# gmum/3d-point-clouds-autocomplete

Measured on AMD Instinct MI355X. Metric: train-step point-clouds/sec at B=64, N=2048 (Chamfer+EMD), higher is better.
Workload: dtype f32 storage / accumulation / results; matrix products formed from f16 x2 (bf16 x3) pieces of the fp32 operands — NOT IEEE-fp32 products: the all-fp32-kernel step is `value_strict_fp32`

## Files before the change

### 3d-point-clouds-autocomplete_amd/csrc/hp_model.h

```cpp
#pragma once

#define HP_MAX_HEADS 8
#define HP_MAX_TN_LAYERS 8

typedef struct HpEncoderWeights {
    const float* conv_w[5];
    const float* conv_b[5];
    const float* fc_w;
    const float* fc_b;
    const float* mu_w;
    const float* mu_b;
    const float* std_w;
    const float* std_b;
} HpEncoderWeights;

typedef struct HpEncoderGrads {
    float* conv_w[5];
    float* conv_b[5];
    float* fc_w;
    float* fc_b;
    float* mu_w;
    float* mu_b;
    float* std_w;
    float* std_b;
} HpEncoderGrads;

typedef struct HpEncoderIO {
    const float* x;
    const HpEncoderWeights* w;
    const float* eps;
    int* argidx;
    float *g, *f, *mu, *lv, *z, *explv, *ws;
    int is_vae;
    int out_ld;
} HpEncoderIO;

typedef struct HpEncoderBwdIO {
    const float* x;
    const HpEncoderWeights* w;
    const float* eps;
    const int* argidx;
    const float *g, *f, *lv;
    const float *grad_out, *grad_mu, *grad_explv;
    const HpEncoderGrads* gr;
    float* ws;
    const float* fwd_ws;
    int is_vae;
    int grad_out_ld;
} HpEncoderBwdIO;

enum { HP_ENC_CONV_PFORMAT = 0, HP_ENC_CONV_SPLIT_F32 = 1, HP_ENC_CONV_GEMM_F32 = 2 };
typedef struct HpEncoderPlan {
    int conv_format;
    int pool_fused;
    int tile_rows;
    int fwd_tails_skinny;
    int bwd_fused;
    int bwd_splits;
    int bwd_tails_skinny[2];
} HpEncoderPlan;

typedef struct HpHyperWeights {
    const float* trunk_w[5];
    const float* trunk_b[5];
    int n_heads;
    int head_out[HP_MAX_HEADS];
    const float* head_w[HP_MAX_HEADS];
    const float* head_b[HP_MAX_HEADS];
} HpHyperWeights;

typedef struct HpHyperGrads {
    float* trunk_w[5];
    float* trunk_b[5];
    float* head_w[HP_MAX_HEADS];
    float* head_b[HP_MAX_HEADS];
} HpHyperGrads;

enum { HP_HEADS_FWD_STREAM = 0, HP_HEADS_FWD_GEMM = 1, HP_HEADS_FWD_PER_HEAD = 2 };
enum { HP_HEADS_DW_DIRECT = 0, HP_HEADS_DW_GEMM = 1, HP_HEADS_DW_PER_HEAD = 2, HP_HEADS_DW_SKIPPED = 3 };
typedef struct HpHeadsPlan {
    int fwd_route;
    int dw_route;
    int dw_rows_route;
} HpHeadsPlan;

#ifdef __cplusplus
bool hp_heads_dw_fast_ok(int cols, const float* t5, const float* out);
bool hp_heads_fwd_enabled();
int hp_heads_fwd_set(int on);
long hp_heads_fwd_ws_floats();
bool hp_heads_fwd_ok(int B, int N, int K, const float* t5, const float* W, const float* ws);
int hp_heads_fwd(int B, int N, const float* t5, const float* W, const float* bias, float* theta, int theta_ld, float* ws,
                 hipStream_t stream);
int hp_heads_dw_launch(int Kc, int rows, int r0, const float* dtheta, int theta_ld, const float* t5, int cols, float* dW,
                       float* db, hipStream_t stream);
#endif
```

### 3d-point-clouds-autocomplete_amd/csrc/model.hip

```cpp
#include "hp_common.h"
#include "hp_gemm.h"
#include "hp_conv_split.h"
#include "hp_model.h"
#include "hp_skinny.h"
#include "hp_enc_bwd.h"
#include <algorithm>
#include <cstdlib>

extern "C" int hp_gemm_f32(const HpGemmDesc* d, hipStream_t stream);
extern "C" int hp_gemm_tile_rows(const HpGemmDesc* d);
extern "C" int hp_colsum_f32(int batch, int M, int N, const float* X, long sXz, int ldx, const float* mask, long sMaskz,
                             int ldmask, float* out, long sOz, float* ws, hipStream_t stream);

namespace {

constexpr int kEnc[6] = {3, 64, 128, 256, 512, 512};
constexpr int kTrunk[5] = {64, 128, 512, 1024, 2048};
constexpr long kSplitWs = 4L << 20;

#define TRY(x)            \
    do {                  \
        int _rc = (x);    \
        if (_rc) return _rc; \
    } while (0)
// ... 977 lines not shown
                                        enc_tail_backward_program(B, out_size, 1, &t[z], pr) == 0 && hp_skinny_check(&pr) == 0;
        }
    }
    if (plan->bwd_fused) {
        HpSkProgram pr;
        const int ok = ask && enc_tail_backward_program(B, out_size, n, t, pr) == 0 && hp_skinny_check(&pr) == 0;
        for (int z = 0; z < n; ++z) plan->bwd_tails_skinny[z] = ok;
    }
    return 0;
}

namespace {
template <typename P>
bool heads_contiguous(P const* hw, P const* hb, const int* out, int n) {
    for (int h = 0; h + 1 < n; ++h)
        if (hw[h + 1] != hw[h] + (long)out[h] * 2048 || hb[h + 1] != hb[h] + out[h]) return false;
    return n > 0;
}

int trunk_forward_skinny(int B, int in_size, const float* latent, const HpHyperWeights* w, float* t, float* slabs,
                         hipStream_t stream) {
    if (B > 64 || in_size % 32) return -2;
    HpSkProgram pr{};
    HpSkSrc src{};
    src.p = latent; src.S = 1; src.ld = in_size;
    float* tl = t;
    float* sl = slabs;
    int kin = in_size;
    for (int l = 0; l < 5; ++l) {
        const int N = kTrunk[l];
        const int S = sk_ranges(kin, N / 32, 4);
        HpSkOp& op = pr.op[pr.nops++];
        op.type = HP_SK_F; op.phase = l;
        op.a = src;
        op.w = w->trunk_w[l]; op.w_ld = kin;
        op.M = B; op.N = N; op.K = kin; op.CL = kin / S;
        op.out_ld = N;
        HpSkSrc next{};
        next.ld = N;
        if (S == 1) {
            op.out = tl; op.out_bias = w->trunk_b[l]; op.out_relu = l < 4;
            next.p = tl; next.S = 1;
        } else {
            op.out = sl; op.out_slab = 64L * N;
            next.p = sl; next.slab = 64L * N; next.S = S; next.bias = w->trunk_b[l]; next.relu = l < 4;
            next.mat = tl; next.ldmat = N;
            sl += (long)S * 64 * N;
            if (sl - slabs > kSplitWs) return -2;
        }
        src = next;
        kin = N;
        tl += (long)B * N;
    }
    if (src.S > 1) {
        HpSkOp& op = pr.op[pr.nops++];
        op.type = HP_SK_FIN; op.phase = 5;
        op.out = src.mat; op.out_ld = src.ldmat;
        src.mat = nullptr;
        op.a = src;
        op.M = B; op.N = 2048; op.K = 1;
    }
    return hp_skinny_run(&pr, stream);
}

int trunk_backward_skinny(int B, int in_size, const float* latent, const HpHyperWeights* w, const float* const* act,
                          float* const* dt, const HpHyperGrads* gr, float* grad_latent, float* slabs, hipStream_t stream) {
    if (B > 64 || in_size % 32) return -2;
    HpSkProgram pr{};
    HpSkSrc src{};
    src.p = dt[4]; src.S = 1; src.ld = kTrunk[4];
    float* sl = slabs;
    int phase = 0;
    auto dw_op = [&](int l) {
        HpSkOp& op = pr.op[pr.nops++];
        op.type = HP_SK_W; op.phase = phase;
        op.a.p = dt[l]; op.a.S = 1; op.a.ld = kTrunk[l];
        op.w = l ? act[l - 1] : latent; op.w_ld = l ? kTrunk[l - 1] : in_size;
        op.out = gr->trunk_w[l]; op.out_ld = op.w_ld; op.rsum = gr->trunk_b[l];
        op.M = B; op.N = kTrunk[l]; op.K = op.w_ld;
    };
    for (int l = 4; l >= 0; --l, ++phase) {
        const int N = kTrunk[l], K = l ? kTrunk[l - 1] : in_size;
        if (l == 0 && !grad_latent) {
            HpSkOp& op = pr.op[pr.nops++];
            op.type = HP_SK_FIN; op.phase = phase;
            op.out = src.mat; op.out_ld = src.ldmat;
            src.mat = nullptr;
            op.a = src;
            op.M = B; op.N = N; op.K = 1;
        } else {
            const int S = sk_ranges(N, K / 32, 4);
            HpSkOp& op = pr.op[pr.nops++];
            op.type = HP_SK_X; op.phase = phase;
            op.a = src;
            op.w = w->trunk_w[l]; op.w_ld = K;
            op.M = B; op.N = N; op.K = K; op.CL = N / S;
            op.out_ld = K;
            HpSkSrc next{};
            next.ld = K;
            if (l == 0) {
                if (S == 1) {
                    op.out = grad_latent;
                } else {
                    op.out = sl; op.out_slab = 64L * K;
                    next.p = sl; next.slab = 64L * K; next.S = S;
                    sl += (long)S * 64 * K;
                }
            } else {
                op.out = sl; op.out_slab = 64L * K;
                next.p = sl; next.slab = 64L * K; next.S = S;
                next.mask = act[l - 1]; next.ldm = K; next.mat = dt[l - 1]; next.ldmat = K;
                sl += (long)S * 64 * K;
            }
            if (sl - slabs > kSplitWs) return -2;
            src = next;
        }
        if (l == 4) dw_op(4);
        else if (l <= 2) dw_op(l + 1);
    }
    if (grad_latent && src.p && src.S > 1) {
        HpSkOp& op = pr.op[pr.nops++];
        op.type = HP_SK_FIN; op.phase = phase;
        op.a = src;
        op.out = grad_latent; op.out_ld = in_size;
        op.M = B; op.N = in_size; op.K = 1;
    }
    dw_op(0);
    return hp_skinny_run(&pr, stream);
}

template <typename T>
inline T* hyper_splitws(T* t, int B) { return t + ((long)B * (64 + 128 + 512 + 1024 + 2048) + 3) / 4 * 4; }
inline int heads_total(const HpHyperWeights* w) {
    int total = 0;
    for (int hd = 0; hd < w->n_heads; ++hd) total += w->head_out[hd];
    return total;
}
int heads_fwd_route(int B, const HpHyperWeights* w, const float* t) {
    if (!heads_contiguous(w->head_w, w->head_b, w->head_out, w->n_heads)) return HP_HEADS_FWD_PER_HEAD;
    const float* t5 = t + (long)B * (64 + 128 + 512 + 1024);
    return hp_heads_fwd_enabled() && hp_heads_fwd_ws_floats() <= kSplitWs &&
                   hp_heads_fwd_ok(B, heads_total(w), 2048, t5, w->head_w[0], hyper_splitws(t, B))
               ? HP_HEADS_FWD_STREAM : HP_HEADS_FWD_GEMM;
}
int heads_dw_route(const HpHyperWeights* w, const HpHyperGrads* gr, const float* t5) {
    const bool skip_dw = gr->head_w[0] == nullptr;
    bool gb_contig = true;
    for (int h = 0; h + 1 < w->n_heads; ++h) gb_contig = gb_contig && gr->head_b[h + 1] == gr->head_b[h] + w->head_out[h];
    const bool w_contig = heads_contiguous(w->head_w, w->head_b, w->head_out, w->n_heads);
    if (skip_dw) return gb_contig && w_contig ? HP_HEADS_DW_SKIPPED : -1;
    if (!w_contig || !heads_contiguous(gr->head_w, gr->head_b, w->head_out, w->n_heads)) return HP_HEADS_DW_PER_HEAD;
    return hp_heads_dw_fast_ok(2048, t5, gr->head_w[0]) ? HP_HEADS_DW_DIRECT : HP_HEADS_DW_GEMM;
}
int heads_dw_rows_route(const float* t5_all, const float* dW_rows) {
    return hp_heads_dw_fast_ok(2048, t5_all, dW_rows) ? HP_HEADS_DW_DIRECT : HP_HEADS_DW_GEMM;
}
}

HP_API long hp_hypernet_saved_floats(int B) { return (long)B * (64 + 128 + 512 + 1024 + 2048) + kSplitWs + 64; }
HP_API long hp_hypernet_backward_workspace_floats(int B) { return (long)B * (64 + 128 + 512 + 1024 + 2048) + kSplitWs + 64; }

HP_API int hp_hypernet_set_heads_stream(int on) { return hp_heads_fwd_set(on); }

HP_API int hp_hypernet_forward(int B, int in_size, const float* latent, const HpHyperWeights* w, float* t, float* theta,
                               int theta_ld, hipStream_t stream) {
    HP_CHECK_ARG(B > 0 && in_size > 0 && latent && w && t && theta && w->n_heads > 0 && w->n_heads <= HP_MAX_HEADS);
    Op op{stream, hyper_splitws(t, B)};
    const float* in = latent;
    int kin = in_size;
    float* tl = t;
    int sk = hp_skinny_enabled() ? trunk_forward_skinny(B, in_size, latent, w, t, op.splitws, stream) : -2;
    if (sk != -2) {
        TRY(sk);
        in = t + (long)B * (64 + 128 + 512 + 1024);
    } else {
        for (int l = 0; l < 5; ++l) {
            TRY(op.lin_fwd(in, 0, kin, w->trunk_w[l], 0, w->trunk_b[l], 0, tl, 0, kTrunk[l], B, kTrunk[l], kin, 1, l < 4));
            in = tl;
            kin = kTrunk[l];
            tl += (long)B * kTrunk[l];
        }
    }
    const int total = heads_total(w);
    HP_CHECK_ARG(total <= theta_ld);
    switch (heads_fwd_route(B, w, t)) {
    case HP_HEADS_FWD_STREAM:
        TRY(hp_heads_fwd(B, total, in, w->head_w[0], w->head_b[0], theta, theta_ld, op.splitws, stream));
        break;
    case HP_HEADS_FWD_GEMM:
        TRY(op.lin_fwd(in, 0, 2048, w->head_w[0], 0, w->head_b[0], 0, theta, 0, theta_ld, B, total, 2048, 1, false));
        break;
    default: {
        int off = 0;
        for (int hd = 0; hd < w->n_heads; ++hd) {
            TRY(op.lin_fwd(in, 0, 2048, w->head_w[hd], 0, w->head_b[hd], 0, theta + off, 0, theta_ld, B, w->head_out[hd], 2048,
                           1, false));
            off += w->head_out[hd];
        }
    }
    }
    HP_RETURN_LAST_ERROR();
}

namespace {
int hypernet_backward_impl(int B, int in_size, const float* latent, const HpHyperWeights* w, const float* t, const float* grad_theta,
                           int theta_ld, const HpHyperGrads* gr, float* grad_latent, float* ws, hipStream_t stream, hipStream_t after);
}
HP_API int hp_hypernet_backward(int B, int in_size, const float* latent, const HpHyperWeights* w, const float* t,
                                const float* grad_theta, int theta_ld, const HpHyperGrads* gr, float* grad_latent, float* ws,
                                hipStream_t stream) {
    return hypernet_backward_impl(B, in_size, latent, w, t, grad_theta, theta_ld, gr, grad_latent, ws, stream, nullptr);
}
HP_API int hp_hypernet_backward_ordered(int B, int in_size, const float* latent, const HpHyperWeights* w, const float* t,
                                        const float* grad_theta, int theta_ld, const HpHyperGrads* gr, float* grad_latent, float* ws,
                                        hipStream_t stream, hipStream_t after) {
    return hypernet_backward_impl(B, in_size, latent, w, t, grad_theta, theta_ld, gr, grad_latent, ws, stream, after);
}
namespace {
int hypernet_backward_impl(int B, int in_size, const float* latent, const HpHyperWeights* w, const float* t, const float* grad_theta,
                           int theta_ld, const HpHyperGrads* gr, float* grad_latent, float* ws, hipStream_t stream, hipStream_t after) {
    HP_CHECK_ARG(B > 0 && in_size > 0 && latent && w && t && grad_theta && gr && ws);
    const float* act[5];
    {
        const float* tl = t;
        for (int l = 0; l < 5; ++l) {
            act[l] = tl;
            tl += (long)B * kTrunk[l];
        }
    }
    float* p = ws;
    float* dt[5];
    for (int l = 0; l < 5; ++l) {
        dt[l] = p;
        p += (long)B * kTrunk[l];
    }
    Op op{stream, p};
    int off = 0;
    const int total = heads_total(w);
    const int route = heads_dw_route(w, gr, act[4]);
    HP_CHECK_ARG(route >= 0);
    const bool fused = route != HP_HEADS_DW_PER_HEAD;
    if (fused) {
        if (route == HP_HEADS_DW_DIRECT) {
            TRY(hp_heads_dw_launch(B, total, 0, grad_theta, theta_ld, act[4], 2048, gr->head_w[0], gr->head_b[0], stream));
        } else if (route == HP_HEADS_DW_GEMM)
            TRY(op.lin_dw(grad_theta, 0, theta_ld, act[4], 0, 2048, gr->head_w[0], 0, B, total, 2048, 1, gr->head_b[0]));
        else if (gr->head_b[0])
            TRY(op.colsum(grad_theta, 0, theta_ld, B, total, 1, gr->head_b[0], 0));
        TRY(op.lin_dx(grad_theta, 0, theta_ld, w->head_w[0], 0, dt[4], 0, 2048, B, total, 2048, 1, nullptr, 0, 0, nullptr, 2048));
    }
    for (int hd = 0; hd < w->n_heads && !fused; ++hd) {
        const int nh = w->head_out[hd];
        TRY(op.lin_dw(grad_theta + off, 0, theta_ld, act[4], 0, 2048, gr->head_w[hd], 0, B, nh, 2048, 1, gr->head_b[hd]));
        TRY(op.lin_dx(grad_theta + off, 0, theta_ld, w->head_w[hd], 0, dt[4], 0, 2048, B, nh, 2048, 1, nullptr, 0, 0,
                      hd ? dt[4] : nullptr, 2048));
        off += nh;
    }
    if (after && after != stream) TRY(hp_order_streams(stream, after));
    {
        const int sk = hp_skinny_enabled() ? trunk_backward_skinny(B, in_size, latent, w, act, dt, gr, grad_latent, p, stream) : -2;
        if (sk != -2) return sk ? sk : (int)hipGetLastError();
    }
    for (int l = 4; l >= 0; --l) {
        const float* below = l ? act[l - 1] : latent;
        const int kin = l ? kTrunk[l - 1] : in_size;
        TRY(op.lin_dw(dt[l], 0, kTrunk[l], below, 0, kin, gr->trunk_w[l], 0, B, kTrunk[l], kin, 1, gr->trunk_b[l]));
        if (l > 0)
            TRY(op.lin_dx(dt[l], 0, kTrunk[l], w->trunk_w[l], 0, dt[l - 1], 0, kin, B, kTrunk[l], kin, 1, act[l - 1], 0, kin,
                          nullptr, 0));
        else if (grad_latent)
            TRY(op.lin_dx(dt[0], 0, kTrunk[0], w->trunk_w[0], 0, grad_latent, 0, kin, B, kTrunk[0], kin, 1, nullptr, 0, 0,
                          nullptr, 0));
    }
    HP_RETURN_LAST_ERROR();
}
}

HP_API long hp_hypernet_t5_offset(int B) { return (long)B * (64 + 128 + 512 + 1024); }
HP_API long hp_hypernet_heads_dw_workspace_floats(void) { return kSplitWs + 64; }
HP_API int hp_hypernet_heads_dw_rows(int Kc, int rows, int r0, const float* dtheta_all, int theta_ld, const float* t5_all,
                                     float* dW_rows, float* ws, hipStream_t stream) {
    HP_CHECK_ARG(Kc > 0 && rows >= 0 && r0 >= 0 && r0 + rows <= theta_ld && dtheta_all && t5_all && ws);
    if (rows == 0) return 0;
    HP_CHECK_ARG(dW_rows);
    if (heads_dw_rows_route(t5_all, dW_rows) == HP_HEADS_DW_DIRECT)
        return hp_heads_dw_launch(Kc, rows, r0, dtheta_all, theta_ld, t5_all, 2048, dW_rows, nullptr, stream);
    Op op{stream, ws};
    TRY(op.lin_dw(dtheta_all + r0, 0, theta_ld, t5_all, 0, 2048, dW_rows, 0, Kc, rows, 2048, 1));
    HP_RETURN_LAST_ERROR();
}

HP_API int hp_hypernet_heads_plan(int B, const HpHyperWeights* w, const HpHyperGrads* gr, const float* t, const float* dW_rows,
                                  HpHeadsPlan* plan) {
    HP_CHECK_ARG(B > 0 && w && t && plan && w->n_heads > 0 && w->n_heads <= HP_MAX_HEADS);
    const float* t5 = t + hp_hypernet_t5_offset(B);
    plan->fwd_route = heads_fwd_route(B, w, t);
    plan->dw_route = gr ? heads_dw_route(w, gr, t5) : -1;
    plan->dw_rows_route = dW_rows ? heads_dw_rows_route(t5, dW_rows) : -1;
    return gr && plan->dw_route < 0 ? -1 : 0;
}

namespace {
struct TnLayout {
    int nl;
    int cin[HP_MAX_TN_LAYERS], cout[HP_MAX_TN_LAYERS];
    long woff[HP_MAX_TN_LAYERS], boff[HP_MAX_TN_LAYERS];
    long total, act_per_point;
};
bool tn_layout(int n_hidden, const int* channels, TnLayout* L) {
    if (n_hidden < 1 || n_hidden + 1 > HP_MAX_TN_LAYERS) return false;
    L->nl = n_hidden + 1;
    long off = 0;
    L->act_per_point = 0;
    for (int l = 0; l < L->nl; ++l) {
        L->cin[l] = l ? channels[l - 1] : 3;
        L->cout[l] = l < n_hidden ? channels[l] : 3;
        L->woff[l] = off;
        off += (long)L->cin[l] * L->cout[l];
        L->boff[l] = off;
        off += L->cout[l];
        if (l < n_hidden) L->act_per_point += channels[l];
    }
    L->total = off;
    return true;
}
}

HP_API long hp_target_theta_size(int n_hidden, const int* channels) {
    TnLayout L;
    return tn_layout(n_hidden, channels, &L) ? L.total : -1;
}
HP_API long hp_target_saved_floats(int B, int N, int n_hidden, const int* channels) {
    TnLayout L;
    return tn_layout(n_hidden, channels, &L) ? (long)B * N * L.act_per_point : -1;
}
HP_API long hp_target_backward_workspace_floats(int B, int N, int n_hidden, const int* channels) {
    TnLayout L;
    return tn_layout(n_hidden, channels, &L) ? (long)B * N * L.act_per_point + kSplitWs + 64 : -1;
}

HP_API int hp_target_forward(int B, int N, int n_hidden, const int* channels, const float* theta, int theta_ld,
                             const float* pts, float* acts, float* y, hipStream_t stream) {
    TnLayout L;
    HP_CHECK_ARG(B > 0 && N > 0 && theta && pts && acts && y && tn_layout(n_hidden, channels, &L) && L.total <= theta_ld);
    Op op{stream, nullptr};
    const float* in = pts;
    float* a = acts;
    for (int l = 0; l < L.nl; ++l) {
        const bool last = (l == L.nl - 1);
        float* out = last ? y : a;
        TRY(op.lin_fwd(in, (long)N * L.cin[l], L.cin[l], theta + L.woff[l], theta_ld, theta + L.boff[l], theta_ld, out,
                       (long)N * L.cout[l], L.cout[l], N, L.cout[l], L.cin[l], B, !last));
        in = out;
        if (!last) a += (long)B * N * L.cout[l];
    }
    HP_RETURN_LAST_ERROR();
}

HP_API int hp_target_backward(int B, int N, int n_hidden, const int* channels, const float* theta, int theta_ld,
                              const float* pts, const float* acts, const float* grad_y, float* grad_theta, float* ws,
                              hipStream_t stream) {
    TnLayout L;
    HP_CHECK_ARG(B > 0 && N > 0 && theta && pts && acts && grad_y && grad_theta && ws && tn_layout(n_hidden, channels, &L) &&
                 L.total <= theta_ld);
    const float* act[HP_MAX_TN_LAYERS];
    float* dl[HP_MAX_TN_LAYERS];
    {
        const float* a = acts;
        float* p = ws;
        for (int l = 0; l < n_hidden; ++l) {
            act[l] = a;
            dl[l] = p;
            a += (long)B * N * L.cout[l];
            p += (long)B * N * L.cout[l];
        }
        ws = p;
    }
    Op op{stream, ws};
    const float* d = grad_y;
    for (int l = L.nl - 1; l >= 0; --l) {
        const float* below = l ? act[l - 1] : pts;
        const int cin = L.cin[l], cout = L.cout[l];
        TRY(op.lin_dw(d, (long)N * cout, cout, below, (long)N * cin, cin, grad_theta + L.woff[l], theta_ld, N, cout, cin, B,
                      grad_theta + L.boff[l], theta_ld));
        if (l > 0) {
            TRY(op.lin_dx(d, (long)N * cout, cout, theta + L.woff[l], theta_ld, dl[l - 1], (long)N * cin, cin, N, cout, cin, B,
                          act[l - 1], (long)N * cin, cin, nullptr, 0));
            d = dl[l - 1];
        }
    }
    HP_RETURN_LAST_ERROR();
}
```

### include/hyperpocket_hip.h

```cpp
#ifndef HYPERPOCKET_HIP_H
#define HYPERPOCKET_HIP_H

#ifdef __cplusplus
extern "C" {
#endif

typedef struct ihipStream_t* hpStream_t;


int hp_nndistance(int b, int n, const float* xyz, int m, const float* xyz2, float* result, int* result_i,
                  float* result2, int* result2_i, hpStream_t stream);

int hp_nn_set_queries_per_lane(int r);
int hp_nn_queries_per_lane(int b, int n, int m);

int hp_nndistancegrad(int b, int n, const float* xyz1, int m, const float* xyz2, const float* grad_dist1,
                      const int* idx1, const float* grad_dist2, const int* idx2, float* grad_xyz1, float* grad_xyz2,
                      hpStream_t stream);

int hp_approxmatch(int b, int n, int m, const float* xyz1, const float* xyz2, float* match, float* temp,
                   hpStream_t stream);
long hp_approxmatch_workspace_floats(int b, int n, int m);
int hp_approxmatch_ws(int b, int n, int m, const float* xyz1, const float* xyz2, float* match, float* temp, float* ws,
                      hpStream_t stream);
// ... 37 lines not shown

int hp_emd_pairs(int na, int n, const float* A, int nb, int m, const float* B, int pairs, const int* pair_ab,
                 float* temp, float* ws, float* partials, float* cost, hpStream_t stream);

#define HP_OCCUPANCY_MAX_R 64
int hp_occupancy_grid(int S, int n, const float* clouds, int R, const float* axis, const unsigned int* columns,
                      int cells, int* counters, int* clouds_hit, int* nonfinite, hpStream_t stream);
int hp_occupancy_cells_host(long count, const float* points, int R, const float* axis, const unsigned int* columns,
                            int* cell_out);

#define HP_GEMM_BIAS 1
#define HP_GEMM_RELU 2
#define HP_GEMM_MASK 4
#define HP_GEMM_ADD 8
#define HP_GEMM_ROWSUM 32
#define HP_GEMM_COLMAX 16

typedef struct HpGemmDesc {
    const float* A;
    const float* B;
    float* C;
    const float* bias;
    const float* mask;
    const float* add;
    float* ws;
    long sAz, sBz, sCz, sBiasz, sMaskz, sAddz;
    long sAi, sAk, sBk, sBj;
    int ldc, ldmask, ldadd;
    int M, N, K, batch;
    int ksplit;
    int flags;
    float* cmax;
    int* cidx;
    int group_rows;
    float* rsum;
    long sRsumz;
    const int* dyn_count;
    int dyn_kind;
} HpGemmDesc;

long hp_gemm_workspace_floats(const HpGemmDesc* d);
int hp_gemm_tile_rows(const HpGemmDesc* d);
int hp_gemm_plan(const HpGemmDesc* d, int* tile, int* mode);
int hp_gemm_f32(const HpGemmDesc* d , hpStream_t stream);
long hp_colsum_workspace_floats(int batch, int M, int N);
int hp_colsum_f32(int batch, int M, int N, const float* X, long sXz, int ldx, const float* mask, long sMaskz,
                  int ldmask, float* out, long sOz, float* ws , hpStream_t stream);

#define HP_MAX_HEADS 8
#define HP_MAX_TN_LAYERS 8

typedef struct HpEncoderWeights {
    const float* conv_w[5];
    const float* conv_b[5];
    const float* fc_w;
    const float* fc_b;
    const float* mu_w;
    const float* mu_b;
    const float* std_w;
    const float* std_b;
} HpEncoderWeights;

typedef struct HpEncoderGrads {
    float* conv_w[5];
    float* conv_b[5];
    float* fc_w;
    float* fc_b;
    float* mu_w;
    float* mu_b;
    float* std_w;
    float* std_b;
} HpEncoderGrads;

typedef struct HpHyperWeights {
    const float* trunk_w[5];
    const float* trunk_b[5];
    int n_heads;
    int head_out[HP_MAX_HEADS];
    const float* head_w[HP_MAX_HEADS];
    const float* head_b[HP_MAX_HEADS];
} HpHyperWeights;

typedef struct HpHyperGrads {
    float* trunk_w[5];
    float* trunk_b[5];
    float* head_w[HP_MAX_HEADS];
    float* head_b[HP_MAX_HEADS];
} HpHyperGrads;

long hp_encoder_forward_workspace_floats(int B, int Np);
int hp_encoder_forward(int B, int Np, const float* x, const HpEncoderWeights* w, int out_size, int is_vae,
                       const float* eps, int* argidx, float* g, float* f, float* mu, float* lv, float* z, float* explv,
                       float* ws, hpStream_t stream);
typedef struct HpEncoderIO {
    const float* x;
    const HpEncoderWeights* w;
    const float* eps;
    int* argidx;
    float *g, *f, *mu, *lv, *z, *explv, *ws;
    int is_vae;
    int out_ld;
} HpEncoderIO;
int hp_encoder_forward_pair(int B, int Np, int out_size, const HpEncoderIO* io , hpStream_t stream);
int hp_encoder_workspace_to_f32(int B, int Np, float* ws, hpStream_t stream);
int hp_conv_presplit_set(int on);
long hp_gemm_pp_workspace_floats(long M, int N, int K);
int hp_gemm_pp_prepare(long M, int N, int K, int xcb, const float* X, const float* W, float* ws, hpStream_t stream);
int hp_gemm_pp_run(long M, int N, int K, int xcb, const float* bias, int relu, int mode, int group_rows, float* ws, hpStream_t stream);
int hp_gemm_pp_unpack(long M, int N, int K, const float* ws, float* C, hpStream_t stream);
int hp_gemm_pp_partials(long M, int N, int K, const float* ws, float* cmax, int* cidx, hpStream_t stream);
long hp_encoder_backward_workspace_floats(int B, int out_size);
int hp_encoder_backward(int B, int Np, const float* x, const HpEncoderWeights* w, int out_size, int is_vae,
                        const float* eps, const int* argidx, const float* g, const float* f, const float* lv,
                        const float* grad_out, const float* grad_mu, const float* grad_explv, const HpEncoderGrads* grads,
                        float* ws, const float* fwd_ws, int dedup, hpStream_t stream);
int hp_encoder_backward_ld(int B, int Np, const float* x, const HpEncoderWeights* w, int out_size, int is_vae,
                           const float* eps, const int* argidx, const float* g, const float* f, const float* lv,
                           const float* grad_out, int grad_out_ld, const float* grad_mu, const float* grad_explv,
                           const HpEncoderGrads* grads, float* ws, const float* fwd_ws, int dedup, hpStream_t stream);
typedef struct HpEncoderBwdIO {
    const float* x;
    const HpEncoderWeights* w;
    const float* eps;
    const int* argidx;
    const float *g, *f, *lv;
    const float *grad_out, *grad_mu, *grad_explv;
    const HpEncoderGrads* gr;
    float* ws;
    const float* fwd_ws;
    int is_vae;
    int grad_out_ld;
} HpEncoderBwdIO;
int hp_encoder_backward_pair(int B, int Np, int out_size, const HpEncoderBwdIO* io , int dedup, hpStream_t stream);
enum { HP_ENC_CONV_PFORMAT = 0, HP_ENC_CONV_SPLIT_F32 = 1, HP_ENC_CONV_GEMM_F32 = 2 };
typedef struct HpEncoderPlan {
    int conv_format;
    int pool_fused;
    int tile_rows;
    int fwd_tails_skinny;
    int bwd_fused;
    int bwd_splits;
    int bwd_tails_skinny[2];
} HpEncoderPlan;
int hp_encoder_plan(int B, int Np, int out_size, int n, const int* is_vae, const int* ld, int aligned, int dedup,
                    HpEncoderPlan* plan);
int hp_encoder_backward_set_fused(int on);
int hp_encoder_backward_set_chain_f16(int on);
int hp_conv_split_set(int on);
long hp_gemm_f16x2_workspace_floats(long M, int N, int K);
int hp_gemm_f16x2_prepare(long M, int N, int K, const float* X, const float* W, float* ws, hpStream_t stream);
int hp_gemm_f16x2_run(long M, int N, int K, const float* X, const float* bias, float* C, int relu, const float* ws, hpStream_t stream);

int hp_hypernet_set_heads_stream(int on);
long hp_hypernet_saved_floats(int B);
int hp_hypernet_forward(int B, int in_size, const float* latent, const HpHyperWeights* w, float* t, float* theta,
                        int theta_ld, hpStream_t stream);
long hp_hypernet_backward_workspace_floats(int B);
int hp_hypernet_backward(int B, int in_size, const float* latent, const HpHyperWeights* w, const float* t,
                         const float* grad_theta, int theta_ld, const HpHyperGrads* grads, float* grad_latent ,
                         float* ws, hpStream_t stream);
int hp_hypernet_backward_ordered(int B, int in_size, const float* latent, const HpHyperWeights* w, const float* t,
                                 const float* grad_theta, int theta_ld, const HpHyperGrads* grads, float* grad_latent ,
                                 float* ws, hpStream_t stream, hpStream_t after);
long hp_hypernet_t5_offset(int B);
long hp_hypernet_heads_dw_workspace_floats(void);
int hp_hypernet_heads_dw_rows(int Kc, int rows, int r0, const float* dtheta_all, int theta_ld, const float* t5_all,
                              float* dW_rows, float* ws, hpStream_t stream);
enum { HP_HEADS_FWD_STREAM = 0, HP_HEADS_FWD_GEMM = 1, HP_HEADS_FWD_PER_HEAD = 2 };
enum { HP_HEADS_DW_DIRECT = 0, HP_HEADS_DW_GEMM = 1, HP_HEADS_DW_PER_HEAD = 2, HP_HEADS_DW_SKIPPED = 3 };
typedef struct HpHeadsPlan {
    int fwd_route;
    int dw_route;
    int dw_rows_route;
} HpHeadsPlan;
int hp_hypernet_heads_plan(int B, const HpHyperWeights* w, const HpHyperGrads* grads , const float* t,
                           const float* dW_rows , HpHeadsPlan* plan);

int hp_hypernet_heads_dw_adam(int Kc, int rows, int r0, const float* dtheta_all, int theta_ld, const float* t5_all,
                              float* W_rows, float* m_rows, float* v_rows, float lr, float beta1, float beta2, float eps,
                              int step, hpStream_t stream);
int hp_hypernet_heads_dw_adam_bg(int Kc, int rows, int r0, const float* dtheta_all, int theta_ld, const float* t5_all,
                                 float* W_rows, float* m_rows, float* v_rows, float lr, float beta1, float beta2, float eps,
                                 int step, int cus, hpStream_t stream);

int hp_skinny_set_enabled(int on);
long hp_skinny_programs_run(void);

long hp_target_theta_size(int n_hidden, const int* channels);
long hp_target_saved_floats(int B, int N, int n_hidden, const int* channels);
int hp_target_forward(int B, int N, int n_hidden, const int* channels, const float* theta, int theta_ld, const float* pts,
                      float* acts, float* y, hpStream_t stream);
long hp_target_backward_workspace_floats(int B, int N, int n_hidden, const int* channels);
int hp_target_backward(int B, int N, int n_hidden, const int* channels, const float* theta, int theta_ld, const float* pts,
                       const float* acts, const float* grad_y, float* grad_theta, float* ws, hpStream_t stream);

int hp_target_fused_supported(int n_hidden, const int* channels);
long hp_target_fused_workspace_floats(int B, int N);
int hp_target_fused_set_f16(int on);
int hp_target_fused_forward(int B, int N, const float* theta, int theta_ld, const float* pts, float* y, hpStream_t stream);
int hp_target_fused_backward(int B, int N, const float* theta, int theta_ld, const float* pts, const float* grad_y,
                             float* grad_theta, float* ws, hpStream_t stream);

int hp_sample_points(long total, float coef, unsigned long long seed, unsigned long long offset, float* out,
                     hpStream_t stream);
int hp_slice_clouds(int B, int N, int target, const float* pts, unsigned long long seed, int max_rounds, float* part_a,
                    float* part_b, float* plane, int* status, hpStream_t stream);
int hp_slice_clouds_planes(int B, int N, int target, const float* pts, const double* planes, int R, float* part_a,
                           float* part_b, int* plane_idx, int* status, hpStream_t stream);
long hp_make_batch_workspace_bytes(int B, int N);
int hp_make_batch(int M, int N, int target, const float* clouds, int B, const int* ids, const long long* streams,
                  const int* degrees, const float* rot, unsigned long long seed, int max_candidates, int groups,
                  float* existing, float* missing, float* gt, float* plane, int* index, int* failed, void* ws,
                  hpStream_t stream);
#define HP_SCAN_MAX_POINTS (1 << 22)
int hp_scan_boxes(int S, const float* points, const long long* offsets, float* center , float* scale ,
                  hpStream_t stream);
int hp_prepare_scans(int B, const float* points, const long long* offsets, int S, const int* ids, const long long* streams,
                     unsigned long long seed, int target, int replace, const float* center, const float* scale, float* out,
                     int* index, int* failed, hpStream_t stream);
int hp_restore_scans(int K, int N, const float* completions, const float* s_scale, const float* center, const float* scale,
                     float* out, hpStream_t stream);
#define HP_FPS_MAX_POINTS 8192
int hp_farthest_points(int B, int P, const float* clouds, const int* counts, const int* start, int k, int* index,
                       float* radius2, int* failed, hpStream_t stream);
int hp_farthest_points_plan(int P, int* threads, int* points_per_lane);
#define HP_KNN_MAX_POINTS 65536
int hp_knn_points(int S, const float* points, const long long* offsets, const float* queries, const long long* query_offsets,
                  int k, int exclude_self, int* index , float* dist2 , hpStream_t stream);
int hp_knn_points_plan(int k, int* instance_k, int* threads, int* tile);
int hp_scan_outliers(int S, const float* points, const long long* offsets, int k, float ratio, unsigned char* keep ,
                     float* mean_dist , int* kept , hpStream_t stream);
#define HP_CLUSTER_MAX_POINTS 32768
int hp_scan_clusters(int S, const float* points, const long long* offsets, float radius, int max_points,
                     int* label , int* size , int* clusters , int* largest ,
                     hpStream_t stream);
int hp_scan_clusters_plan(int max_points, int* threads, int* tile, int* lds_bytes);
#define HP_PLANE_MAX_TRIALS 4096
long hp_scan_plane_workspace_bytes(int S, int trials);
int hp_scan_plane_plan(int trials, int* threads, int* rows_per_lane, int* trial_tile);
int hp_scan_plane(int S, const float* points, const long long* offsets, const long long* streams ,
                  unsigned long long seed, int trials, float threshold, int min_inliers, float min_share,
                  int* trial , int* inliers , int* found , int* sample ,
                  float* sample_plane , unsigned char* inlier , long long* moments ,
                  int* shift , void* ws, hpStream_t stream);
int hp_scan_plane_side(int S, const float* points, const long long* offsets, const float* planes , float threshold,
                       float* dist , unsigned char* keep , int* kept , hpStream_t stream);
#define HP_VOXEL_GRID_HALF (1 << 20)
long hp_scan_voxels_workspace_bytes(long long T, int slots_per_row);
int hp_scan_voxels_plan(int* threads, int* rows_per_lane);
int hp_scan_voxels(int S, long long T, const float* points, const long long* offsets, const float* voxel ,
                   const float* origin , int keep_mode, int slots_per_row, int* label ,
                   int* size , unsigned char* keep , int* kept , int* beyond , void* ws,
                   hpStream_t stream);
#define HP_ALIGN_MAX_POINTS 65536
#define HP_ALIGN_MAX_HYPOTHESES 64
long hp_scan_align_workspace_bytes(int S, int H);
int hp_scan_align_plan(int H, int* threads, int* rows_per_lane, int* hypothesis_group, int* tile);
int hp_scan_align_step(int S, int H, long long T, const float* points, const long long* offsets, long long U,
                       const float* tpoints, const long long* toffsets, const float* transforms , float max_dist,
                       const float* anchor , const int* shift , long long* moments ,
                       int* index , float* dist2 , hpStream_t stream);
long hp_scan_align_plane_workspace_bytes(int S, int H);
int hp_scan_align_plane_plan(int H, int* threads, int* rows_per_lane, int* hypothesis_group, int* tile);
int hp_scan_align_plane_step(int S, int H, long long T, const float* points, const long long* offsets, long long U,
                             const float* tpoints, const long long* toffsets, const float* tnormals ,
                             const float* transforms , float max_dist, const float* anchor ,
                             const int* shift , long long* moments , int* index ,
                             float* dist2 , hpStream_t stream);
int hp_scan_normals_plan(int k, int* instance_k, int* threads, int* sweeps);
int hp_scan_normals(int S, const float* points, const long long* offsets, int k, const int* index ,
                    const float* viewpoints , float* normal , float* curvature ,
                    int* count , hpStream_t stream);
#define HP_AXIS_SPLIT_MAX_POINTS 8192
int hp_axis_split(int B, int n, const float* clouds , int axis, int k,
                  float* lower , float* upper , int* order ,
                  hpStream_t stream);
#define HP_MESH_MAX_FACES 32768
int hp_mesh_sample(int K, int V, const float* verts, int F, const int* faces, int n, unsigned long long seed,
                   const long long* streams , float* points , int* face ,
                   double* area , int* failed , void* ws, hpStream_t stream);
long hp_mesh_sample_workspace_bytes(int K, int F, int n);
int hp_mesh_sample_plan(int K, int F, int n, int* threads, int* slices, int* in_lds);
int hp_mesh_sample_set_slices(int s);
int hp_mesh_sample_set_lds_faces(int faces);
int hp_mesh_normals(int K, int V, const float* verts, int F, const int* faces, const int* vf_offsets, const int* vf_faces,
                    float* face_normal , float* vertex_normal , hpStream_t stream);
int hp_kld_forward(long n, int batch, const float* explv, const float* mu, float* out, hpStream_t stream);
int hp_kld_backward(long n, int batch, const float* explv, const float* mu, const float* grad_out, float* grad_explv,
                    float* grad_mu, hpStream_t stream);
int hp_step_losses(int b, const float* cd, const float* kld, const float* cost, float c_cd, float c_emd, float* out ,
                   hpStream_t stream);

int hp_adam_step(long n, float* p, const float* g, float* m, float* v, float lr, float beta1, float beta2, float eps,
                 int step, float grad_scale, hpStream_t stream);

#define HP_TSNE_MAX_POINTS 16384
int hp_pairwise_sqdist(int n, int d, const float* X, long ldx, float* D , hpStream_t stream);
int hp_pairwise_sqdist_plan(int n, int d, int* tile, int* kchunk);
long hp_tsne_affinities_workspace_floats(int n);
int hp_tsne_affinities(int n, const float* D, float perplexity, float* P , float* beta ,
                       int* steps , float* ws, hpStream_t stream);
int hp_tsne_gradient(int n, const float* P, float exaggeration, const float* Y , float* rowacc ,
                     float* kl , hpStream_t stream);
int hp_tsne_update(int n, const float* rowacc, float* Y, float* update, float* gains, float momentum, float lr,
                   float min_gain, float* grad , hpStream_t stream);
int hp_tsne_descend(int n, const float* P, float* Y, float* update, float* gains, float* rowacc, int it0, int iters,
// ... 26 lines not shown
```

Measured before the change: 28590.

## Add streaming split-K MFMA kernel for hypernetwork heads input-gradient

```diff
diff --git a/3d-point-clouds-autocomplete_amd/csrc/heads_dx.hip b/3d-point-clouds-autocomplete_amd/csrc/heads_dx.hip
--- /dev/null
+++ b/3d-point-clouds-autocomplete_amd/csrc/heads_dx.hip
@@ -0,0 +1,188 @@
+#include "hp_common.h"
+#include "hp_model.h"
+#include <type_traits>
+
+namespace {
+
+typedef float f32x16 __attribute__((ext_vector_type(16)));
+
+constexpr int kCols = 2048, kTiles = kCols / 32;
+constexpr int kWaves = 4, kThreads = kWaves * 64;
+constexpr int kChunk = 32;
+constexpr int kRing = 3;
+constexpr int kWStage = kChunk * 128;
+constexpr int kDStage = 64 * 32 * 4;
+constexpr int kStage = kWStage + kDStage;
+constexpr int kWaveLds = kRing * kStage;
+constexpr int kLds = kWaves * kWaveLds;
+constexpr int kMaxSplits = 16;
+constexpr long kSlab = 64L * kCols;
+
+__device__ __forceinline__ void glds16(const void* sbase, unsigned voff, unsigned lds_dst) {
+    unsigned keep;
+    asm volatile("s_mov_b32 %0, m0\n\ts_mov_b32 m0, %3\n\ts_nop 0\n\tglobal_load_lds_dwordx4 %1, %2\n\ts_mov_b32 m0, %0"
+                 : "=&s"(keep)
+                 : "v"(voff), "s"(sbase), "s"(lds_dst)
+                 : "memory");
+}
+
+template <int NT>
+__global__ __launch_bounds__(kThreads, 1) void heads_dx_kernel(int B, int N, int L, int splits, const float* __restrict__ dth,
+                                                                int theta_ld, const float* __restrict__ W, float* __restrict__ slabs) {
+    constexpr int kD = 4 * NT, kDma = 4 + kD;
+    __shared__ __attribute__((aligned(1024))) unsigned char lds[kLds];
+    const int tid = threadIdx.x, lane = tid & 63, w = __builtin_amdgcn_readfirstlane(tid >> 6), i = lane & 31, h = lane >> 5;
+    const int ct = blockIdx.x % kTiles, split = (blockIdx.x / kTiles) * kWaves + w;
+    if (split >= splits) return;
+    const int r_lo = min(split * L, N), r_hi = min(r_lo + L, N);
+    const int nch = (r_hi - r_lo + kChunk - 1) / kChunk;
+    auto uniform_ptr = [](const void* q) {
+        const unsigned long long p = reinterpret_cast<unsigned long long>(q);
+        const unsigned lo = __builtin_amdgcn_readfirstlane((unsigned)p), hi = __builtin_amdgcn_readfirstlane((unsigned)(p >> 32));
+        return reinterpret_cast<const void*>(((unsigned long long)hi << 32) | lo);
+    };
+    const void* wbase = uniform_ptr(W);
+    const unsigned long long dptr = reinterpret_cast<unsigned long long>(dth);
+    const void* dbase = uniform_ptr(reinterpret_cast<const void*>(dptr & ~15ull));
+    const unsigned boff = __builtin_amdgcn_readfirstlane((unsigned)(dptr & 15) >> 2);
+    const unsigned jmax = (boff + (unsigned)(B - 1) * (unsigned)theta_ld + (unsigned)(N - 1)) >> 2;
+    const unsigned wave_lds = __builtin_amdgcn_readfirstlane((unsigned)(size_t)lds + (unsigned)(w * kWaveLds));
+    const int wrow = lane >> 3;
+    const unsigned wcol = (unsigned)(ct * 128 + (lane & 7) * 16);
+    unsigned ec[kD];
+#pragma unroll
+    for (int p = 0; p < kD; ++p) {
+        const int c = 8 * p + (lane >> 3), piece = ((lane & 7) - (c >> 1)) & 7;
+        ec[p] = boff + (unsigned)min(c, B - 1) * (unsigned)theta_ld + 4u * (unsigned)piece;
+    }
+    auto issue_w = [&](int n0, unsigned st, int j) {
+        const int row = min(n0 + 8 * j + wrow, N - 1);
+        glds16(wbase, (unsigned)row * (unsigned)(kCols * 4) + wcol, st + j * 1024);
+    };
+    auto issue_d = [&](int n0, unsigned st, int p) {
+        const unsigned piece = min((ec[p] + (unsigned)n0) >> 2, jmax);
+        glds16(dbase, piece << 4, st + kWStage + p * 1024);
+    };
+    const int rb = h * 512 + i * 4;
+    int ra[NT], ph[NT], rot[NT];
+#pragma unroll
+    for (int t = 0; t < NT; ++t) {
+        const int c = 32 * t + i;
+        ra[t] = kWStage + c * 128;
+        ph[t] = (int)((boff + (unsigned)c * (unsigned)theta_ld) & 3) + 4 * h;
+        rot[t] = ph[t] + 4 * ((c >> 1) & 7);
+    }
+    f32x16 acc[NT] = {};
+    if (nch > 0) {
+        int slot_w = 0;
+#pragma unroll 1
+        for (int c = 0; c < 2; ++c) {
+            const int nw = r_lo + min(c, nch - 1) * kChunk, nd = r_lo + c * kChunk;
+            const unsigned st = wave_lds + (unsigned)(slot_w * kStage);
+#pragma unroll
+            for (int j = 0; j < 4; ++j) issue_w(nw, st, j);
+#pragma unroll
+            for (int p = 0; p < kD; ++p) issue_d(nd, st, p);
+            slot_w = slot_w == kRing - 1 ? 0 : slot_w + 1;
+        }
+        int slot_r = 0;
+#pragma unroll 1
+        for (int c = 0; c < nch; ++c) {
+            asm volatile("s_waitcnt vmcnt(%0)" ::"n"(kDma) : "memory");
+            const int n0 = r_lo + c * kChunk;
+            const int nw2 = r_lo + min(c + 2, nch - 1) * kChunk, nd2 = r_lo + min(c + 2, nch) * kChunk;
+            const unsigned st2 = wave_lds + (unsigned)(slot_w * kStage);
+            const unsigned char* st = lds + w * kWaveLds + slot_r * kStage;
+            const unsigned char* stn = lds + w * kWaveLds + (slot_r == kRing - 1 ? 0 : slot_r + 1) * kStage;
+            const int lim = r_hi - n0 - 4 * h;
+            float av[2][4][NT], bv[2][4];
+            auto read_group = [&](int g, float (&a)[4][NT], float (&b)[4]) {
+#pragma unroll
+                for (int s = 0; s < 4; ++s) {
+                    const int r0 = 8 * g + s;
+                    b[s] = *reinterpret_cast<const float*>(st + rb + r0 * 128);
+#pragma unroll
+                    for (int t = 0; t < NT; ++t) {
+                        const unsigned char* base = (g == 3 && ph[t] + r0 >= 32) ? stn : st;
+                        a[s][t] = *reinterpret_cast<const float*>(base + ra[t] + ((rot[t] + r0) & 31) * 4);
+                    }
+                }
+            };
+            auto contract = [&](auto ragged) {
+                read_group(0, av[0], bv[0]);
+#pragma unroll
+                for (int g = 0; g < 4; ++g) {
+                    if (g + 1 < 4) {
+                        if (g + 1 == 3) asm volatile("s_waitcnt vmcnt(8)" ::: "memory");
+                        read_group(g + 1, av[(g + 1) & 1], bv[(g + 1) & 1]);
+                    }
+                    __builtin_amdgcn_sched_barrier(0);
+#pragma unroll
+                    for (int s = 0; s < 4; ++s) {
+                        const int q = 4 * g + s;
+#pragma unroll
+                        for (int t = 0; t < NT; ++t) {
+                            const bool zero = decltype(ragged)::value && 8 * g + s >= lim;
+                            const float a = zero ? 0.f : av[g & 1][s][t], b = zero ? 0.f : bv[g & 1][s];
+                            acc[t] = __builtin_amdgcn_mfma_f32_32x32x2f32(a, b, acc[t], 0, 0, 0);
+                            __builtin_amdgcn_sched_barrier(0);
+                            if (t == 0 && q < kDma) {
+                                if (q < 4) issue_w(nw2, st2, q);
+                                else issue_d(nd2, st2, q - 4);
+                                __builtin_amdgcn_sched_barrier(0);
+                            }
+                        }
+                    }
+                }
+            };
+            if (n0 + kChunk > r_hi) contract(std::true_type{});
+            else contract(std::false_type{});
+            slot_w = slot_w == kRing - 1 ? 0 : slot_w + 1;
+            slot_r = slot_r == kRing - 1 ? 0 : slot_r + 1;
+        }
+    }
+    float* out = slabs + (long)split * kSlab + ct * 32 + i;
+#pragma unroll
+    for (int t = 0; t < NT; ++t)
+#pragma unroll
+        for (int e = 0; e < 16; ++e) {
+            const int row = t * 32 + (e & 3) + 8 * (e >> 2) + 4 * h;
+            if (row < B) out[(long)row * kCols] = acc[t][e];
+        }
+    asm volatile("s_waitcnt vmcnt(0)" ::: "memory");
+}
+
+__global__ __launch_bounds__(256) void heads_dx_finish_kernel(int B, int S, const float* __restrict__ slabs, float* __restrict__ out) {
+    const int idx = blockIdx.x * 256 + threadIdx.x;
+    if (idx >= B * (kCols / 4)) return;
+    const float4* p = reinterpret_cast<const float4*>(slabs) + idx;
+    float4 v = S <= 8 ? p[0] : make_float4(0.f, 0.f, 0.f, 0.f);
+    for (int s = S <= 8 ? 1 : 0; s < S; ++s) {
+        const float4 t = p[(long)s * (kSlab / 4)];
+        v = make_float4(v.x + t.x, v.y + t.y, v.z + t.z, v.w + t.w);
+    }
+    reinterpret_cast<float4*>(out)[idx] = v;
+}
+
+hp::Switch g_heads_dx("HP_HEADS_DX", 1);
+
+}
+
+bool hp_heads_dx_enabled() { return g_heads_dx.get() != 0; }
+int hp_heads_dx_set(int on) { return g_heads_dx.set(on); }
+long hp_heads_dx_ws_floats(int splits) { return (long)splits * kSlab; }
+bool hp_heads_dx_ok(int B, int N, int K, int theta_ld, int splits, int rows, const float* dtheta, const float* W, const float* slabs,
+                    const float* dt5) {
+    auto a16 = [](const void* p) { return (reinterpret_cast<uintptr_t>(p) & 15) == 0; };
+    return B >= 1 && B <= 64 && K == kCols && N >= 1 && theta_ld >= N && (long)N * K * 4 < (1L << 32) &&
+           (long)B * theta_ld * 4 < (1L << 32) && splits >= 1 && splits <= kMaxSplits && rows > 0 && rows % kChunk == 0 &&
+           (long)splits * rows >= N && dtheta && a16(W) && a16(slabs) && a16(dt5);
+}
+int hp_heads_dx(int B, int N, int splits, int rows, const float* dtheta, int theta_ld, const float* W, float* slabs, float* dt5,
+                hipStream_t stream) {
+    const dim3 grid(kTiles * ((splits + kWaves - 1) / kWaves));
+    if (B > 32) hipLaunchKernelGGL(heads_dx_kernel<2>, grid, dim3(kThreads), 0, stream, B, N, rows, splits, dtheta, theta_ld, W, slabs);
+    else hipLaunchKernelGGL(heads_dx_kernel<1>, grid, dim3(kThreads), 0, stream, B, N, rows, splits, dtheta, theta_ld, W, slabs);
+    hipLaunchKernelGGL(heads_dx_finish_kernel, dim3((B * (kCols / 4) + 255) / 256), dim3(256), 0, stream, B, splits, slabs, dt5);
+    HP_RETURN_LAST_ERROR();
+}
diff --git a/3d-point-clouds-autocomplete_amd/csrc/hp_model.h b/3d-point-clouds-autocomplete_amd/csrc/hp_model.h
--- a/3d-point-clouds-autocomplete_amd/csrc/hp_model.h
+++ b/3d-point-clouds-autocomplete_amd/csrc/hp_model.h
@@ -92,6 +92,13 @@
 bool hp_heads_fwd_ok(int B, int N, int K, const float* t5, const float* W, const float* ws);
 int hp_heads_fwd(int B, int N, const float* t5, const float* W, const float* bias, float* theta, int theta_ld, float* ws,
                  hipStream_t stream);
+bool hp_heads_dx_enabled();
+int hp_heads_dx_set(int on);
+long hp_heads_dx_ws_floats(int splits);
+bool hp_heads_dx_ok(int B, int N, int K, int theta_ld, int splits, int rows, const float* dtheta, const float* W, const float* slabs,
+                    const float* dt5);
+int hp_heads_dx(int B, int N, int splits, int rows, const float* dtheta, int theta_ld, const float* W, float* slabs, float* dt5,
+                hipStream_t stream);
 int hp_heads_dw_launch(int Kc, int rows, int r0, const float* dtheta, int theta_ld, const float* t5, int cols, float* dW,
                        float* db, hipStream_t stream);
 #endif
diff --git a/3d-point-clouds-autocomplete_amd/csrc/model.hip b/3d-point-clouds-autocomplete_amd/csrc/model.hip
--- a/3d-point-clouds-autocomplete_amd/csrc/model.hip
+++ b/3d-point-clouds-autocomplete_amd/csrc/model.hip
@@ -1153,6 +1153,18 @@
     if (!w_contig || !heads_contiguous(gr->head_w, gr->head_b, w->head_out, w->n_heads)) return HP_HEADS_DW_PER_HEAD;
     return hp_heads_dw_fast_ok(2048, t5, gr->head_w[0]) ? HP_HEADS_DW_DIRECT : HP_HEADS_DW_GEMM;
 }
+struct HeadsDxPlan {
+    int splits, rows;
+    bool stream;
+};
+HeadsDxPlan heads_dx_plan(int B, int total, int theta_ld, const float* grad_theta, const float* W, const float* slabs, const float* dt5) {
+    HeadsDxPlan r;
+    r.splits = pick_ksplit(B, 2048, total, 1);
+    r.rows = std::max(32, ((total + r.splits - 1) / r.splits + 31) / 32 * 32);
+    r.stream = hp_heads_dx_enabled() && r.splits <= 16 && hp_heads_dx_ws_floats(r.splits) <= kSplitWs &&
+               hp_heads_dx_ok(B, total, 2048, theta_ld, r.splits, r.rows, grad_theta, W, slabs, dt5);
+    return r;
+}
 int heads_dw_rows_route(const float* t5_all, const float* dW_rows) {
     return hp_heads_dw_fast_ok(2048, t5_all, dW_rows) ? HP_HEADS_DW_DIRECT : HP_HEADS_DW_GEMM;
 }
@@ -1248,7 +1260,11 @@
             TRY(op.lin_dw(grad_theta, 0, theta_ld, act[4], 0, 2048, gr->head_w[0], 0, B, total, 2048, 1, gr->head_b[0]));
         else if (gr->head_b[0])
             TRY(op.colsum(grad_theta, 0, theta_ld, B, total, 1, gr->head_b[0], 0));
-        TRY(op.lin_dx(grad_theta, 0, theta_ld, w->head_w[0], 0, dt[4], 0, 2048, B, total, 2048, 1, nullptr, 0, 0, nullptr, 2048));
+        const HeadsDxPlan dx = heads_dx_plan(B, total, theta_ld, grad_theta, w->head_w[0], p, dt[4]);
+        if (dx.stream)
+            TRY(hp_heads_dx(B, total, dx.splits, dx.rows, grad_theta, theta_ld, w->head_w[0], p, dt[4], stream));
+        else
+            TRY(op.lin_dx(grad_theta, 0, theta_ld, w->head_w[0], 0, dt[4], 0, 2048, B, total, 2048, 1, nullptr, 0, 0, nullptr, 2048));
     }
     for (int hd = 0; hd < w->n_heads && !fused; ++hd) {
         const int nh = w->head_out[hd];
@@ -1288,6 +1304,21 @@
         return hp_heads_dw_launch(Kc, rows, r0, dtheta_all, theta_ld, t5_all, 2048, dW_rows, nullptr, stream);
     Op op{stream, ws};
     TRY(op.lin_dw(dtheta_all + r0, 0, theta_ld, t5_all, 0, 2048, dW_rows, 0, Kc, rows, 2048, 1));
+    HP_RETURN_LAST_ERROR();
+}
+
+HP_API int hp_hypernet_set_heads_dx(int on) { return hp_heads_dx_set(on); }
+
+HP_API int hp_hypernet_heads_dx_route(int B, int N, int theta_ld, const float* dtheta, const float* W, const float* dt5, const float* ws) {
+    return B > 0 && N > 0 && heads_dx_plan(B, N, theta_ld, dtheta, W, ws, dt5).stream ? 1 : 0;
+}
+HP_API int hp_hypernet_heads_dx(int B, int N, const float* dtheta, int theta_ld, const float* W, float* dt5, float* ws,
+                                hipStream_t stream) {
+    HP_CHECK_ARG(B > 0 && N > 0 && theta_ld >= N && dtheta && W && dt5 && ws);
+    const HeadsDxPlan dx = heads_dx_plan(B, N, theta_ld, dtheta, W, ws, dt5);
+    if (dx.stream) return hp_heads_dx(B, N, dx.splits, dx.rows, dtheta, theta_ld, W, ws, dt5, stream);
+    Op op{stream, ws};
+    TRY(op.lin_dx(dtheta, 0, theta_ld, W, 0, dt5, 0, 2048, B, N, 2048, 1, nullptr, 0, 0, nullptr, 2048));
     HP_RETURN_LAST_ERROR();
 }
 
diff --git a/include/hyperpocket_hip.h b/include/hyperpocket_hip.h
--- a/include/hyperpocket_hip.h
+++ b/include/hyperpocket_hip.h
@@ -213,6 +213,9 @@
 int hp_gemm_f16x2_run(long M, int N, int K, const float* X, const float* bias, float* C, int relu, const float* ws, hpStream_t stream);
 
 int hp_hypernet_set_heads_stream(int on);
+int hp_hypernet_set_heads_dx(int on);
+int hp_hypernet_heads_dx_route(int B, int N, int theta_ld, const float* dtheta, const float* W, const float* dt5, const float* ws);
+int hp_hypernet_heads_dx(int B, int N, const float* dtheta, int theta_ld, const float* W, float* dt5, float* ws, hpStream_t stream);
 long hp_hypernet_saved_floats(int B);
 int hp_hypernet_forward(int B, int in_size, const float* latent, const HpHyperWeights* w, float* t, float* theta,
                         int theta_ld, hpStream_t stream);
```

Result: no change. 28510 (-0.3%).
